# chaobrain/brainevent

Hardware: AMD Instinct MI355X
Metric: synaptic updates/sec (Geff/s), BinaryArray @ CSR scatter (higher is better)
Workload: dtype f32; 1 GPU; BinaryArray(0.01 fire) @ CSR f32 hetero, 1000000 pre x 1000000 post, 10000 synapses/row (0.01 density), route=ScatterPlan; parallelism=post-slice x1, n_post_per_gpu=1000000, n_conn=10000, stored_synapses_total=10000000000, plan_slices=51 x 19608 columns x 5 parts, layout d8 (5 B/entry)

## Files before the change

brainevent_amd/csrc/be_csr_plan.hip:

```cpp
#include "be_csr_shared.h"
#include <climits>
#include <cstring>
#ifndef BE_BLOCK_AUX
#define BE_BLOCK_AUX 2
#endif
constexpr int kD8NtMinBlock = 160;

namespace {

constexpr int kMaxSlices = 4096;

__host__ __device__ __forceinline__ uint32_t plan_group(bool homo) { return homo ? 8u : 4u; }
__host__ __device__ __forceinline__ uint32_t plan_block_units(uint32_t n_groups, bool homo) {
  const uint32_t bytes = n_groups * (homo ? 16u : 24u);
  return (bytes + 127u) >> 7;
}

__global__ void __launch_bounds__(256) k_plan_count(const int32_t* __restrict__ indices, RowPtr rp, int64_t m,
                                                    uint32_t slice_width, int n_slices, int homo, uint2* __restrict__ seg) {
  __shared__ uint32_t hist[kMaxSlices];
  for (int64_t r = blockIdx.x; r < m; r += gridDim.x) {
    for (int s = threadIdx.x; s < n_slices; s += blockDim.x) hist[s] = 0;
    __syncthreads();
    const int64_t b = rp.at(r), e = rp.at(r + 1);
// ... 133 lines not shown
#pragma unroll
    for (int off = 32; off > 0; off >>= 1) {
      const uint32_t o = __shfl_down(my_max, off, 64);
      my_max = o > my_max ? o : my_max;
    }
    if (lane_id() == 0 && my_max != 0) atomicMax(maxabs_bits, my_max);
#pragma unroll
    for (int off = 32; off > 0; off >>= 1) {
      const uint32_t o = __shfl_down(my_min, off, 64);
      my_min = o < my_min ? o : my_min;
    }
    if (lane_id() == 0 && my_min != 0xffffffffu) atomicMin(maxabs_bits + 1, my_min);
  }
}

template <int FUSED>
__device__ __forceinline__ uint32_t fused_word(const void* __restrict__ spikes, int64_t gw, int64_t m) {
  uint32_t w = 0;
  if (FUSED == 1) {
    w = static_cast<const uint32_t*>(spikes)[gw];
  } else {
    const uint8_t* sp = static_cast<const uint8_t*>(spikes) + gw * 32;
    if (gw * 32 + 32 <= m) {
      const uint4 a = reinterpret_cast<const uint4*>(sp)[0], b = reinterpret_cast<const uint4*>(sp)[1];
      const uint32_t v[8] = {a.x, a.y, a.z, a.w, b.x, b.y, b.z, b.w};
#pragma unroll
      for (int q = 0; q < 8; ++q)
#pragma unroll
        for (int e = 0; e < 4; ++e) w |= (((v[q] >> (8 * e)) & 0xffu) != 0u ? 1u : 0u) << (4 * q + e);
    } else {
      for (int e = 0; e < 32 && gw * 32 + e < m; ++e) w |= (sp[e] != 0 ? 1u : 0u) << e;
    }
  }
  const int64_t left = m - gw * 32;
  return left >= 32 ? w : (left > 0 ? (w & ((1u << (uint32_t)left) - 1u)) : 0u);
}

__device__ __forceinline__ uint32_t block_scan_total_1024(uint32_t v, uint32_t* wave_tot , uint32_t* total) {
  const int lane = threadIdx.x & 63, wave = threadIdx.x >> 6;
  uint32_t incl = v;
#pragma unroll
  for (int off = 1; off < 64; off <<= 1) {
    const uint32_t t = __shfl_up(incl, off, 64);
    if (lane >= off) incl += t;
  }
  if (lane == 63) wave_tot[wave] = incl;
  __syncthreads();
  uint32_t base = 0, t = 0;
#pragma unroll
  for (int w = 0; w < 16; ++w) {
    const uint32_t x = wave_tot[w];
    t += x;
    if (w < wave) base += x;
  }
  *total = t;
  return base + incl;
}

template <int FUSED>
__device__ __forceinline__ uint32_t build_part_list(const void* __restrict__ spikes, int64_t m, int part, int parts,
                                                    uint32_t* lds_list, uint32_t lds_cap, uint32_t* glob_list,
                                                    uint32_t* wave_tot , const uint32_t** list_out) {
  const int64_t n_words = (m + 31) >> 5;
  const int64_t n_stripes = (n_words + 31) >> 5;
  const int64_t my_words = part < n_stripes ? ((n_stripes - part + parts - 1) / parts) * 32 : 0;
  uint32_t* dst = lds_list;
  uint32_t base = 0;
  int buf = 0;
  for (int64_t u0 = 0; u0 < my_words; u0 += 1024) {
    const int64_t u = u0 + threadIdx.x;
    const int64_t gw = ((u >> 5) * parts + part) * 32 + (u & 31);
    uint32_t w = (u < my_words && gw < n_words) ? fused_word<FUSED>(spikes, gw, m) : 0u;
    const uint32_t v = __popc(w);
    uint32_t it_total;
    uint32_t pos = base + block_scan_total_1024(v, wave_tot + 16 * buf, &it_total) - v;
    buf ^= 1;
    if (dst == lds_list && base + it_total > lds_cap) {
      dst = glob_list;
      base = 0;
      u0 = -1024;
      continue;
    }
    while (w) {
      const uint32_t b = __ffs(w) - 1u;
      dst[pos++] = (uint32_t)(gw * 32) + b;
      w &= w - 1u;
    }
    base += it_total;
  }
  __syncthreads();
  *list_out = dst;
  return base;
}

__global__ void __launch_bounds__(256) k_gather_seg(const uint2* __restrict__ seg, const uint32_t* __restrict__ active,
                                                    const uint32_t* __restrict__ n_active_p, int n_slices, int64_t a_stride,
                                                    uint2* __restrict__ dense) {
  __shared__ uint2 tile[64][65];
  const uint32_t n_active = *n_active_p;
  const int lane = threadIdx.x & 63, wave = threadIdx.x >> 6;
  for (uint32_t c = blockIdx.x; (uint64_t)c * 64 < n_active; c += gridDim.x) {
    const uint32_t a0 = c * 64;
    const uint32_t n_here = n_active - a0 < 64u ? n_active - a0 : 64u;
    const uint32_t i_mine = (uint32_t)wave * 16u + (uint32_t)(lane & 15);
    const uint32_t rid = active[a0 + (i_mine < n_here ? i_mine : 0u)];
    for (int s0 = 0; s0 < n_slices; s0 += 64) {
      const int sl = s0 + lane < n_slices ? s0 + lane : n_slices - 1;
// ... 241 lines not shown
  if (L >= n_tasks) return;
  const int part = L / n_slices;
  const int slice = L - part * n_slices;
  if constexpr (FUSED == 0) active += (int64_t)blockIdx.y * active_stride;
  partial += ((int64_t)blockIdx.y * n_tasks + L) * stride;
  {
    uint4* z = reinterpret_cast<uint4*>(smem_raw);
    const int n16 = (int)(((size_t)(S + 1) * sizeof(acc_t) + 15) / 16);
    for (int i = threadIdx.x; i < n16; i += blockDim.x) z[i] = make_uint4(0u, 0u, 0u, 0u);
  }
  __syncthreads();

  __shared__ uint32_t fused_wtot[32];
  uint32_t n_active;
  if constexpr (FUSED == 1 || FUSED == 2) {
    n_active = build_part_list<FUSED>(static_cast<const unsigned char*>(fused_spikes) + (int64_t)blockIdx.y * fused_stride, fused_m,
                                      part, parts, reinterpret_cast<uint32_t*>(smem_raw + list_off), lds_cap,
                                      glob_lists + ((int64_t)blockIdx.y * parts + part) * glob_region, fused_wtot, &active);
  } else {
    n_active = n_active_p[blockIdx.y];
  }
  uint32_t pos_lo = 0;
  if constexpr (FUSED == 3) {
    const uint32_t npp = (n_active + (uint32_t)parts - 1u) / (uint32_t)parts;
    pos_lo = (uint32_t)part * npp;
    const uint32_t hi = pos_lo + npp < n_active ? pos_lo + npp : n_active;
    n_active = hi > pos_lo ? hi : pos_lo;
  }
  const uint2* sp = FUSED == 3 ? seg + (int64_t)slice * glob_region : seg + slice;
  const uint64_t seg_rs = FUSED == 3 ? 1u : (uint64_t)n_slices;
  const int wave = threadIdx.x >> 6, lane = threadIdx.x & 63, nw = blockDim.x >> 6;
  const uint64_t a0 = FUSED == 3 ? (uint64_t)pos_lo + (uint64_t)wave * 64 + lane
                      : FUSED  ? (uint64_t)wave + (uint64_t)nw * lane
// ... 400 lines not shown
  }
#pragma unroll
  for (int off = 32; off > 0; off >>= 1) {
    const uint32_t o = __shfl_down(my_max, off, 64);
    my_max = o > my_max ? o : my_max;
  }
  if (lane_id() == 0 && my_max != 0) atomicMax(maxabs_bits, my_max);
#pragma unroll
  for (int off = 32; off > 0; off >>= 1) {
    const uint32_t o = __shfl_down(my_min, off, 64);
    my_min = o < my_min ? o : my_min;
  }
  if (lane_id() == 0) atomicMin(maxabs_bits + 1, my_min);
}

__device__ __forceinline__ uint32_t wave_incl_scan_u32(uint32_t v) {
  v += (uint32_t)__builtin_amdgcn_update_dpp(0, (int)v, 0x111, 0xf, 0xf, false);
  v += (uint32_t)__builtin_amdgcn_update_dpp(0, (int)v, 0x112, 0xf, 0xf, false);
  v += (uint32_t)__builtin_amdgcn_update_dpp(0, (int)v, 0x114, 0xf, 0xf, false);
  v += (uint32_t)__builtin_amdgcn_update_dpp(0, (int)v, 0x118, 0xf, 0xf, false);
  v += (uint32_t)__builtin_amdgcn_update_dpp(0, (int)v, 0x142, 0xa, 0xf, false);
  v += (uint32_t)__builtin_amdgcn_update_dpp(0, (int)v, 0x143, 0xc, 0xf, false);
  return v;
}

__device__ __forceinline__ void d8_add4(unsigned long long* acc, uint32_t before, uint32_t d, const be_v4u& wv, float scale) {
  const uint32_t c0 = before + (d & 0xffu), c1 = c0 + ((d >> 8) & 0xffu), c2 = c1 + ((d >> 16) & 0xffu), c3 = c2 + (d >> 24);
#ifdef BE_ABL_NOATOMIC
  const unsigned long long v0 = fixed_from_f32(__uint_as_float(wv.x), scale), v1 = fixed_from_f32(__uint_as_float(wv.y), scale),
                           v2 = fixed_from_f32(__uint_as_float(wv.z), scale), v3 = fixed_from_f32(__uint_as_float(wv.w), scale);
  asm volatile("" ::"v"(c0), "v"(c1), "v"(c2), "v"(c3), "v"(v0), "v"(v1), "v"(v2), "v"(v3));
#else
  atomicAdd(&acc[c0], fixed_from_f32(__uint_as_float(wv.x), scale));
  atomicAdd(&acc[c1], fixed_from_f32(__uint_as_float(wv.y), scale));
  atomicAdd(&acc[c2], fixed_from_f32(__uint_as_float(wv.z), scale));
  atomicAdd(&acc[c3], fixed_from_f32(__uint_as_float(wv.w), scale));
#endif
}
__device__ __forceinline__ uint32_t d8_sum4(uint32_t d) { return (d & 0xffu) + ((d >> 8) & 0xffu) + ((d >> 16) & 0xffu) + (d >> 24); }

// ... 156 lines not shown
  using acc_t = unsigned long long;
  extern __shared__ __align__(16) unsigned char smem_raw[];
  acc_t* acc = reinterpret_cast<acc_t*>(smem_raw);
  const int S = cap;
#ifdef BE_PLAN_PROF
  unsigned long long plan_t = __builtin_amdgcn_s_memtime();
#endif
  const int per_xcd = gridDim.x >> 3;
  const int L = (blockIdx.x & 7) * per_xcd + (blockIdx.x >> 3);
  const int n_tasks = n_slices * parts;
  if (L >= n_tasks) return;
  const int part = L / n_slices;
  const int slice = L - part * n_slices;
  if constexpr (FUSED == 0) active += (int64_t)blockIdx.y * active_stride;
  partial += ((int64_t)blockIdx.y * n_tasks + L) * S;
  {
    uint4* z = reinterpret_cast<uint4*>(smem_raw);
    const int n16 = (int)(((size_t)(S + 1) * sizeof(acc_t) + 15) / 16);
    for (int i = threadIdx.x; i < n16; i += blockDim.x) z[i] = make_uint4(0u, 0u, 0u, 0u);
  }
  __syncthreads();
  PLAN_STAMP(0);
  __shared__ uint32_t fused_wtot[32];
  uint32_t n_active;
  if constexpr (FUSED == 1 || FUSED == 2) {
    n_active = build_part_list<FUSED>(static_cast<const unsigned char*>(fused_spikes) + (int64_t)blockIdx.y * fused_stride, fused_m,
                                      part, parts, reinterpret_cast<uint32_t*>(smem_raw + list_off), lds_cap,
                                      glob_lists + ((int64_t)blockIdx.y * parts + part) * glob_region, fused_wtot, &active);
  } else {
    n_active = n_active_p[blockIdx.y];
  }
  uint32_t pos_lo = 0;
  if constexpr (FUSED == 3) {
    const uint32_t npp = (n_active + (uint32_t)parts - 1u) / (uint32_t)parts;
    pos_lo = (uint32_t)part * npp;
    const uint32_t hi = pos_lo + npp < n_active ? pos_lo + npp : n_active;
    n_active = hi > pos_lo ? hi : pos_lo;
  }
  PLAN_STAMP(1);
  const uint2* sp = FUSED == 3 ? seg + (int64_t)slice * glob_region : seg + slice;
  const uint64_t seg_rs = FUSED == 3 ? 1u : (uint64_t)n_slices;
  const int wave = threadIdx.x >> 6, lane = threadIdx.x & 63, nw = blockDim.x >> 6;
  const uint64_t a0 = FUSED == 3 ? (uint64_t)pos_lo + (uint64_t)wave * 64 + lane
                      : FUSED  ? (uint64_t)wave + (uint64_t)nw * lane
                               : (uint64_t)part + (uint64_t)parts * ((uint64_t)wave + (uint64_t)nw * lane);
  const uint64_t a_step = FUSED ? (uint64_t)nw * 64 : (uint64_t)parts * nw * 64;
  if (n_active > pos_lo) {
    const uint64_t last = n_active - 1;
    uint64_t a = a0;
    bool v_n = a < n_active;
    uint32_t r_n = FUSED == 3 ? (uint32_t)(a < last ? a : last) : active[a < last ? a : last];
    a += a_step;
    uint2 sg = sp[(uint64_t)r_n * seg_rs];
    uint32_t st_v = sg.x, n4_v = v_n ? sg.y : 0u;
    bool v_c = v_n;
    v_n = a < n_active;
    r_n = FUSED == 3 ? (uint32_t)(a < last ? a : last) : active[a < last ? a : last];
    a += a_step;
    PLAN_STAMP(2);
    while (__ballot(v_c) != 0ull) {
      const int nvalid = __popcll(__ballot(v_c));
      const uint2 sgn = sp[(uint64_t)r_n * seg_rs];
      const bool v_nn = a < n_active;
      const uint32_t r_nn = FUSED == 3 ? (uint32_t)(a < last ? a : last) : active[a < last ? a : last];
      a += a_step;
      if constexpr (LPB > 0) {
        constexpr int BPI = 64 / LPB;
        constexpr int NGRP = 64 / BPI;
        constexpr int DEPTH = 4;
        QGroupD8 g[NGRP];
#pragma unroll
        for (int q = 0; q < DEPTH; ++q) d8q_issue<LPB>(g[q], q * BPI, nvalid, st_v, n4_v, lane, blob);
#pragma unroll
        for (int q = 0; q < NGRP; ++q) {
          if (q + DEPTH < NGRP) d8q_issue<LPB>(g[q + DEPTH], (q + DEPTH) * BPI, nvalid, st_v, n4_v, lane, blob);
          d8q_consume<LPB>(g[q], acc, lane, scale);
        }
        d8q_tails<LPB>(st_v, n4_v, nvalid, acc, lane, scale, blob);
      } else {
// ... 152 lines not shown
  const int n_tasks = n_slices * parts;
  if (L >= n_tasks) return;
  const int part = L / n_slices;
  const int slice = L - part * n_slices;
  if constexpr (FUSED == 0) active += (int64_t)blockIdx.y * active_stride;
  partial += ((int64_t)blockIdx.y * n_tasks + L) * S;
  {
    uint4* z = reinterpret_cast<uint4*>(smem_raw);
    const int n16 = (int)((size_t)S * 4 / 16);
    for (int i = threadIdx.x; i < n16; i += blockDim.x) z[i] = make_uint4(0u, 0u, 0u, 0u);
  }
  __syncthreads();
  __shared__ uint32_t fused_wtot[32];
  uint32_t n_active;
  if constexpr (FUSED == 1 || FUSED == 2) {
    n_active = build_part_list<FUSED>(static_cast<const unsigned char*>(fused_spikes) + (int64_t)blockIdx.y * fused_stride, fused_m,
                                      part, parts, reinterpret_cast<uint32_t*>(smem_raw + list_off), lds_cap,
                                      glob_lists + ((int64_t)blockIdx.y * parts + part) * glob_region, fused_wtot, &active);
  } else {
    n_active = n_active_p[blockIdx.y];
  }
  uint32_t pos_lo = 0;
  if constexpr (FUSED == 3) {
    const uint32_t npp = (n_active + (uint32_t)parts - 1u) / (uint32_t)parts;
    pos_lo = (uint32_t)part * npp;
    const uint32_t hi = pos_lo + npp < n_active ? pos_lo + npp : n_active;
    n_active = hi > pos_lo ? hi : pos_lo;
  }
  const uint2* sp = FUSED == 3 ? seg + (int64_t)slice * glob_region : seg + slice;
  const uint64_t seg_rs = FUSED == 3 ? 1u : (uint64_t)n_slices;
  const int wave = threadIdx.x >> 6, lane = threadIdx.x & 63, nw = blockDim.x >> 6;
  const uint64_t a0 = FUSED == 3 ? (uint64_t)pos_lo + (uint64_t)wave * 64 + lane
                      : FUSED  ? (uint64_t)wave + (uint64_t)nw * lane
// ... 470 lines not shown
                              (layout == BE_PLAN_H8 && slice_width <= kH8MaxWidth));
}
static inline int64_t cap_of(int slice_shift, int slice_width, int layout, int homo) {
  if (layout == BE_PLAN_D8) return (width_of(slice_shift, slice_width) + 1) & ~1ll;
  if (layout == BE_PLAN_H8) return (width_of(slice_shift, slice_width) + 3) & ~3ll;
  const int64_t w = width_of(slice_shift, slice_width);
  return homo ? (w + 3) & ~3ll : (w + 1) & ~1ll;
}
static inline int64_t lds_slots_of(int slice_shift, int slice_width, int layout, int homo) {
  return layout == BE_PLAN_U16 ? (1ll << slice_shift) : cap_of(slice_shift, slice_width, layout, homo);
}

#define COMMA ,
constexpr int kPreGatherMaxBlock = 64;
constexpr int kPreGatherMinSlices = 40;
constexpr size_t kFusedMinList = 2048;
static inline int64_t fused_region_of(int64_t m, int parts) {
  const int64_t n_stripes = (((m + 31) >> 5) + 31) >> 5;
  return ((n_stripes + parts - 1) / parts) * 1024;
}

int64_t be_scatter_plan_scratch_bytes(int64_t m, int64_t k, int slice_shift, int slice_width) {
  const int64_t n = (int64_t)n_slices_of(k, slice_shift, slice_width) * m;
  const int64_t n_blocks = (n + kScanChunk - 1) / kScanChunk;
  return be_align_up((n_blocks + 2) * 8, 256);
}

static inline unsigned long long* plan_too_long(void* scratch, int64_t m, int n_slices) {
  const int64_t n_blocks = ((int64_t)n_slices * m + kScanChunk - 1) / kScanChunk;
  return reinterpret_cast<unsigned long long*>(static_cast<uint64_t*>(scratch) + n_blocks + 1);
}
// ... 396 lines not shown
                                               int parts, int homo) {
  const int64_t n_slices = n_slices_of(k, slice_shift, slice_width);
  const int64_t acc_bytes = homo ? 4 : 8;
  const int64_t task = std::max<int64_t>(1ll << slice_shift, (width_of(slice_shift, slice_width) + 3) & ~3ll);
  return counts_bytes(n_batch) + n_batch * plan_active_stride(m) * 4 +
         be_align_up(n_batch * n_slices * parts * task * acc_bytes, 256);
}
int64_t be_binary_csrmm_t_plan_workspace_bytes_for(int64_t m, int64_t k, int64_t n_batch, int slice_shift, int slice_width,
                                                   int parts, int homo, int block_hint) {
  const int64_t base = be_binary_csrmm_t_plan_workspace_bytes(m, k, n_batch, slice_shift, slice_width, parts, homo);
  const bool pre = block_hint > 0 && block_hint <= pregather_max_block();
  return base + (pre ? plan_dense_seg_bytes(m, n_slices_of(k, slice_shift, slice_width), n_batch) : 0);
}
int64_t be_binary_csrmv_t_plan_workspace_bytes(int64_t m, int64_t k, int slice_shift, int slice_width, int parts, int homo) {
  return be_binary_csrmm_t_plan_workspace_bytes(m, k, 1, slice_shift, slice_width, parts, homo);
}

int be_binary_csrmm_t_plan(const void* weights, int homo, int wdtype, const void* blob, const void* seg,
                           const void* spikes, int spike_dtype, void* out, int64_t m, int64_t k, int64_t n_batch,
                           int slice_shift, int slice_width, int layout, int block_hint, int parts, int scale_exp,
                           void* workspace, int64_t workspace_bytes, be_stream_t stream) {
  BE_REQUIRE(m > 0 && k > 0 && m <= 0xffffffffll && k <= 0xffffffffll, BE_ERR_INVALID, "bad shape");
  BE_REQUIRE(layout == BE_PLAN_U16 || (layout == BE_PLAN_D8 && !homo) || (layout == BE_PLAN_H8 && homo), BE_ERR_INVALID,
             "bad plan layout");
  BE_REQUIRE(n_batch >= 1 && n_batch <= kMaxBatch, BE_ERR_INVALID, "n_batch out of range");
  BE_REQUIRE(slice_shift >= 4 && slice_shift <= 15, BE_ERR_INVALID, "slice_shift must be in [4, 15]");
  BE_REQUIRE(width_ok(slice_shift, slice_width, layout), BE_ERR_INVALID, "slice_width out of range for this layout");
  BE_REQUIRE(parts >= 1 && parts <= 64, BE_ERR_INVALID, "parts must be in [1, 64]");
  BE_REQUIRE(seg && spikes && out && blob, BE_ERR_INVALID, "null pointer");
  BE_REQUIRE(!homo || weights != nullptr, BE_ERR_INVALID, "missing weights");
// ... 25 lines not shown
    int rc1 = BE_ERR_INVALID;
#define BE_SINGLE(LAY, WT) rc1 = launch_plan_single<LAY, WT>(blob, seg, spikes, spike_dtype, m, k, (int)slots, sc1, isc1, weights, out, lds, st)
#define BE_SINGLE_W(LAY)                                                    \
    switch (wdtype) {                                                        \
      case BE_F32: BE_SINGLE(LAY, float); break;                             \
      case BE_F16: BE_SINGLE(LAY, __half); break;                            \
      case BE_BF16: BE_SINGLE(LAY, __hip_bfloat16); break;                   \
      default: be_set_error("planned scatter: f32 / f16 / bf16 outputs"); rc1 = BE_ERR_UNSUPPORTED; \
    }
    if (lay == 0) { BE_SINGLE_W(0) } else if (lay == 1) { BE_SINGLE_W(1) } else if (lay == 2) { BE_SINGLE_W(2) } else { BE_SINGLE_W(3) }
#undef BE_SINGLE_W
#undef BE_SINGLE
    be_prof_end(prof1, st);
    return rc1;
  }
  static const int fused_off = [] { const char* e = getenv("BE_PLAN_FUSED"); return e && e[0] == '0'; }();
  const size_t lds_room = 160 * 1024 - 1024 - lds;
  int fused = 0;
  if (!fused_off && lds + 1024 <= 160 * 1024 && lds_room >= kFusedMinList * 4) {
    if (spike_dtype == BE_SPIKE_BITS) fused = 1;
    else if (spike_dtype == BE_SPIKE_BOOL && (reinterpret_cast<uintptr_t>(spikes) & 15) == 0 && (n_batch == 1 || m % 16 == 0)) fused = 2;
  }
  const int64_t dense_bytes = plan_dense_seg_bytes(m, n_slices, n_batch);
  if (dense_bytes > 0 && block_hint > 0 && block_hint <= pregather_max_block() &&
      workspace_bytes >= be_binary_csrmm_t_plan_workspace_bytes(m, k, n_batch, slice_shift, slice_width, parts, homo) + dense_bytes)
    fused = 3;
  const uint32_t lds_cap = (fused == 1 || fused == 2) ? (uint32_t)std::min<size_t>(lds_room / 4, 32768) : 0u;
  const uint32_t list_off = (uint32_t)lds;
  const size_t lds_dyn = lds + (size_t)lds_cap * 4;
  const int64_t fused_stride = spike_dtype == BE_SPIKE_BITS ? ((m + 31) / 32) * 4 : m;
  const int64_t glob_region = fused == 3 ? astride : fused_region_of(m, parts);
  ActiveList al{active, count};
  const int pre_mode = fused != 3 ? 0 : (spike_dtype == BE_SPIKE_BITS ? 1 :
                       (spike_dtype == BE_SPIKE_BOOL && (reinterpret_cast<uintptr_t>(spikes) & 15) == 0) ? 2 : 0);
  if (fused == 0 || (fused == 3 && pre_mode == 0)) {
    int rc = be_resolve_active(spikes, spike_dtype, m, n_batch, active, astride, count, st, false, &al);
    if (rc != BE_OK) return rc;
  }
  const void* seg_used = seg;
  if (fused == 3) {
    uint2* dense = reinterpret_cast<uint2*>(static_cast<unsigned char*>(partial) +
                                            be_align_up((int64_t)n_slices * parts * S * (homo ? 4 : 8), 256));
    const unsigned cg_grid = (unsigned)(((m + 15) / 16 + 255) / 256);
    if (pre_mode == 1)
// ... 16 lines not shown
#define BE_FUSED_ARGS spikes, m, fused_stride, list_off, lds_cap, active, glob_region
#define BE_PLAN_LAUNCH(KERN, ...)                                                                              \
  do {                                                                                                         \
    auto kern__ = KERN;                                                                                        \
    BE_HIP(be_allow_lds(reinterpret_cast<const void*>(kern__), (int)lds_dyn));                                 \
    hipLaunchKernelGGL(kern__, grid, block, lds_dyn, st, static_cast<const unsigned char*>(blob),              \
                       static_cast<const uint2*>(seg_used), al.ids, al.count, __VA_ARGS__, BE_FUSED_ARGS);     \
  } while (0)
#define BE_PLAN_BY_FUSED(TMPL_A, TMPL_B, ...)                                                                 \
  do {                                                                                                         \
    if (fused == 1) BE_PLAN_LAUNCH((TMPL_A 1 TMPL_B), __VA_ARGS__);                                           \
    else if (fused == 2) BE_PLAN_LAUNCH((TMPL_A 2 TMPL_B), __VA_ARGS__);                                      \
    else if (fused == 3) BE_PLAN_LAUNCH((TMPL_A 3 TMPL_B), __VA_ARGS__);                                      \
    else BE_PLAN_LAUNCH((TMPL_A 0 TMPL_B), __VA_ARGS__);                                                      \
  } while (0)
  if (layout == BE_PLAN_H8) {
    BE_PLAN_BY_FUSED(k_plan_accumulate_h8<, >, n_slices, (int)S, parts, static_cast<uint32_t*>(partial), astride);
  } else if (homo) {
    uint32_t* pp = static_cast<uint32_t*>(partial);
    if (block_hint > 0 && block_hint <= kSub4MaxBlock) BE_PLAN_BY_FUSED(k_plan_accumulate<true COMMA 4 COMMA, >, n_slices, slice_shift, parts, scale, pp, astride, (int)S);
    else if (block_hint > 0 && block_hint <= kSub8MaxBlock) BE_PLAN_BY_FUSED(k_plan_accumulate<true COMMA 8 COMMA, >, n_slices, slice_shift, parts, scale, pp, astride, (int)S);
    else if (block_hint > 0 && block_hint <= kSub16MaxBlock) BE_PLAN_BY_FUSED(k_plan_accumulate<true COMMA 16 COMMA, >, n_slices, slice_shift, parts, scale, pp, astride, (int)S);
    else if (block_hint > 0 && block_hint <= kSub32MaxBlock) BE_PLAN_BY_FUSED(k_plan_accumulate<true COMMA 32 COMMA, >, n_slices, slice_shift, parts, scale, pp, astride, (int)S);
    else BE_PLAN_BY_FUSED(k_plan_accumulate<true COMMA 0 COMMA, >, n_slices, slice_shift, parts, scale, pp, astride, (int)S);
  } else if (layout == BE_PLAN_D8) {
    unsigned long long* pp = static_cast<unsigned long long*>(partial);
    if (block_hint > 0 && block_hint <= kD8EighthMaxBlock) BE_PLAN_BY_FUSED(k_plan_accumulate_d8<8 COMMA, >, n_slices, (int)S, parts, scale, pp, astride);
    else if (block_hint > 0 && block_hint <= kD8QuarterMaxBlock) BE_PLAN_BY_FUSED(k_plan_accumulate_d8<16 COMMA, >, n_slices, (int)S, parts, scale, pp, astride);
    else if (block_hint >= kD8NtMinBlock) BE_PLAN_BY_FUSED(k_plan_accumulate_d8<0 COMMA, COMMA BE_BLOCK_AUX>, n_slices, (int)S, parts, scale, pp, astride);
    else BE_PLAN_BY_FUSED(k_plan_accumulate_d8<0 COMMA, COMMA 0>, n_slices, (int)S, parts, scale, pp, astride);
  } else {
    unsigned long long* pw = static_cast<unsigned long long*>(partial);
    if (block_hint > 0 && block_hint <= kSubW4MaxBlock) BE_PLAN_BY_FUSED(k_plan_accumulate<false COMMA 4 COMMA, >, n_slices, slice_shift, parts, scale, pw, astride, (int)S);
    else if (block_hint > 0 && block_hint <= kSubW8MaxBlock) BE_PLAN_BY_FUSED(k_plan_accumulate<false COMMA 8 COMMA, >, n_slices, slice_shift, parts, scale, pw, astride, (int)S);
    else if (block_hint > 0 && block_hint <= kSubW16MaxBlock) BE_PLAN_BY_FUSED(k_plan_accumulate<false COMMA 16 COMMA, >, n_slices, slice_shift, parts, scale, pw, astride, (int)S);
    else if (block_hint > 0 && block_hint <= kSubW32MaxBlock) BE_PLAN_BY_FUSED(k_plan_accumulate<false COMMA 32 COMMA, >, n_slices, slice_shift, parts, scale, pw, astride, (int)S);
    else BE_PLAN_BY_FUSED(k_plan_accumulate<false COMMA 0 COMMA, >, n_slices, slice_shift, parts, scale, pw, astride, (int)S);
  }
#undef BE_PLAN_BY_FUSED
#undef BE_PLAN_LAUNCH
#undef BE_FUSED_ARGS
  be_prof_end(prof, st);
  BE_LAUNCH_CHECK();
  const int rgrid = grid_for(k, 256, n_batch >= 8 ? 256 : 2048);
  const int64_t pstride = (int64_t)n_tasks * S;
  BE_DISPATCH_W(wdtype, homo,
                hipLaunchKernelGGL((k_plan_reduce<W, HOMO>), dim3(rgrid, (unsigned)n_batch), dim3(256), 0, st,
                                   static_cast<const typename PlanAcc<HOMO>::type*>(partial), parts, n_slices, (int)S,
                                   (uint32_t)width_of(slice_shift, slice_width), k, inv_scale, static_cast<const W*>(weights), static_cast<W*>(out), pstride, count));
  BE_LAUNCH_CHECK();
  return BE_OK;
}

// ... 10 lines not shown
```

include/brainevent_amd.h:

```cpp
#ifndef BRAINEVENT_AMD_H
#define BRAINEVENT_AMD_H

#include <stdint.h>

#ifdef __cplusplus
extern "C" {
#endif

#define BE_OK 0
#define BE_ERR_INVALID (-1)
#define BE_ERR_WORKSPACE (-2)
#define BE_ERR_HIP (-3)
#define BE_ERR_RANGE (-4)
#define BE_ERR_UNSUPPORTED (-5)

#define BE_F32 0
#define BE_F64 1
#define BE_F16 2
#define BE_BF16 3
#define BE_SPIKE_BOOL 0
#define BE_SPIKE_FLOAT 1
#define BE_SPIKE_BITS 2
#define BE_SPIKE_IDS 3
typedef struct be_spike_ids {
// ... 126 lines not shown
int64_t be_fixed_point_scratch_bytes(int64_t k);
int be_weight_stats(const void* weights, int wdtype, int64_t n, uint32_t* max_bits_host, uint32_t* min_nonzero_bits_host,
                    void* scratch, int64_t scratch_bytes, be_stream_t stream);
int be_fixed_point_exponent(const void* weights, int wdtype, const int32_t* indices, int64_t nnz, int64_t k,
                            int min_weight_bits, int keep_exp, void* scratch, int64_t scratch_bytes, int* scale_exp_host,
                            be_stream_t stream);
int be_scatter_plan_exponent(const void* blob, const void* seg, int64_t m, int64_t k, int slice_shift, int slice_width, int layout,
                             int64_t nnz, const uint32_t* maxabs_bits, int min_weight_bits, int keep_exp, void* scratch,
                             int64_t scratch_bytes, int* scale_exp_host, be_stream_t stream);

int64_t be_binary_csrmv_t_plan_workspace_bytes(int64_t m, int64_t k, int slice_shift, int slice_width, int parts, int homo);
int64_t be_binary_csrmm_t_plan_workspace_bytes(int64_t m, int64_t k, int64_t n_batch, int slice_shift, int slice_width,
                                               int parts, int homo);
int64_t be_binary_csrmm_t_plan_workspace_bytes_for(int64_t m, int64_t k, int64_t n_batch, int slice_shift, int slice_width,
                                                   int parts, int homo, int block_hint);
int be_binary_csrmv_t_plan(const void* weights, int homo, int wdtype, const void* blob, const void* seg,
                           const void* spikes, int spike_dtype, void* out, int64_t m, int64_t k, int slice_shift,
                           int slice_width, int layout, int block_hint, int parts, int scale_exp, void* workspace,
                           int64_t workspace_bytes, be_stream_t stream);
int be_binary_csrmm_t_plan(const void* weights, int homo, int wdtype, const void* blob, const void* seg,
                           const void* spikes_bm, int spike_dtype, void* out_bm, int64_t m, int64_t k, int64_t n_batch,
                           int slice_shift, int slice_width, int layout, int block_hint, int parts, int scale_exp,
                           void* workspace, int64_t workspace_bytes, be_stream_t stream);

int be_binned_bins(int64_t k, int slice_shift, int homo);
int be_binned_set_tuning(int task_groups, int min_tasks);
int be_binned_workspace_status(const void* workspace, int clear, be_stream_t stream);
int be_binned_workspace_audit(const void* workspace, uint64_t* counters_host, be_stream_t stream);
int64_t be_binary_csrmv_t_binned_workspace_bytes(int64_t m, int64_t k, int slice_shift, int64_t bin_capacity);
int be_binary_csrmv_t_binned_workspace_init(void* workspace, int64_t workspace_bytes, int64_t m, int64_t k, int slice_shift,
// ... 187 lines not shown
```

Baseline: 816.3 Geff/s.

## Build compact 16-bit active lists and overlap accumulator zeroing in fused d8 plan

Adds fused modes 4/5 for the wave-level d8 accumulate kernel. In these modes each part's active-row list is kept in LDS as 16-bit offsets plus a few bound markers, which halves LDS use and lets longer lists stay on-chip. The list build now loads several spike words per thread, converts byte spikes to bits with dot4, uses DPP-based wave scans with two 16-bit counts packed per lane, and zeroes the accumulator while the spike loads are in flight. The cost is an extra decode step for every row lookup and more register pressure, and mode selection is moved into a new exported helper.

```diff
diff --git a/brainevent_amd/csrc/be_csr_plan.hip b/brainevent_amd/csrc/be_csr_plan.hip
--- a/brainevent_amd/csrc/be_csr_plan.hip
+++ b/brainevent_amd/csrc/be_csr_plan.hip
@@ -171,83 +171,154 @@
   }
 }
 
-template <int FUSED>
-__device__ __forceinline__ uint32_t fused_word(const void* __restrict__ spikes, int64_t gw, int64_t m) {
+__device__ __forceinline__ uint32_t wave_incl_scan_u32(uint32_t v) {
+  v += (uint32_t)__builtin_amdgcn_update_dpp(0, (int)v, 0x111, 0xf, 0xf, false);
+  v += (uint32_t)__builtin_amdgcn_update_dpp(0, (int)v, 0x112, 0xf, 0xf, false);
+  v += (uint32_t)__builtin_amdgcn_update_dpp(0, (int)v, 0x114, 0xf, 0xf, false);
+  v += (uint32_t)__builtin_amdgcn_update_dpp(0, (int)v, 0x118, 0xf, 0xf, false);
+  v += (uint32_t)__builtin_amdgcn_update_dpp(0, (int)v, 0x142, 0xa, 0xf, false);
+  v += (uint32_t)__builtin_amdgcn_update_dpp(0, (int)v, 0x143, 0xc, 0xf, false);
+  return v;
+}
+
+__device__ __forceinline__ uint32_t block_scan_waves_1024(uint32_t wave_total, int wave , uint32_t* wave_tot ,
+                                                          uint32_t* total) {
+  const int lane = threadIdx.x & 63;
+  if (lane == 0) wave_tot[wave] = wave_total;
+  __syncthreads();
+  const uint32_t x = wave_tot[lane & 15];
+  const uint32_t incl = wave_incl_scan_u32(lane < 16 ? x : 0u);
+  *total = (uint32_t)__builtin_amdgcn_readlane((int)incl, 15);
+  return wave ? (uint32_t)__builtin_amdgcn_readlane((int)incl, wave - 1) : 0u;
+}
+
+template <int SRC> struct ListWords { static constexpr int n = SRC == 1 ? 8 : 7; };
+constexpr int kListBounds = 8;
+
+template <int SRC> struct SpikeRaw { uint32_t w; };
+template <> struct SpikeRaw<2> { uint4 a, b; };
+
+template <int SRC>
+__device__ __forceinline__ void spike_raw_load(SpikeRaw<SRC>& r, const void* __restrict__ spikes, int64_t gw, int64_t m) {
+  if constexpr (SRC == 1) {
+    r.w = static_cast<const uint32_t*>(spikes)[gw];
+  } else {
+    const int64_t last = (m - 1) >> 4, c = gw * 2;
+    const uint4* p = static_cast<const uint4*>(spikes);
+    r.a = p[c];
+    r.b = p[c + 1 < last ? c + 1 : last];
+  }
+}
+
+__device__ __forceinline__ uint32_t nonzero_bytes(uint32_t v) { return (((v & 0x7f7f7f7fu) + 0x7f7f7f7fu) | v) & 0x80808080u; }
+
+template <int SRC>
+__device__ __forceinline__ uint32_t spike_raw_bits(const SpikeRaw<SRC>& r, int64_t gw, int64_t m) {
   uint32_t w = 0;
-  if (FUSED == 1) {
-    w = static_cast<const uint32_t*>(spikes)[gw];
+  if constexpr (SRC == 1) {
+    w = r.w;
   } else {
-    const uint8_t* sp = static_cast<const uint8_t*>(spikes) + gw * 32;
-    if (gw * 32 + 32 <= m) {
-      const uint4 a = reinterpret_cast<const uint4*>(sp)[0], b = reinterpret_cast<const uint4*>(sp)[1];
-      const uint32_t v[8] = {a.x, a.y, a.z, a.w, b.x, b.y, b.z, b.w};
-#pragma unroll
-      for (int q = 0; q < 8; ++q)
-#pragma unroll
-        for (int e = 0; e < 4; ++e) w |= (((v[q] >> (8 * e)) & 0xffu) != 0u ? 1u : 0u) << (4 * q + e);
-    } else {
-      for (int e = 0; e < 32 && gw * 32 + e < m; ++e) w |= (sp[e] != 0 ? 1u : 0u) << e;
+    const uint32_t v[8] = {r.a.x, r.a.y, r.a.z, r.a.w, r.b.x, r.b.y, r.b.z, r.b.w};
+#pragma unroll
+    for (int j = 0; j < 4; ++j) {
+      uint32_t x = __builtin_amdgcn_udot4(nonzero_bytes(v[2 * j]), 0x08040201u, 0u, false);
+      x = __builtin_amdgcn_udot4(nonzero_bytes(v[2 * j + 1]), 0x80402010u, x, false);
+      w |= (x >> 7) << (8 * j);
     }
   }
   const int64_t left = m - gw * 32;
   return left >= 32 ? w : (left > 0 ? (w & ((1u << (uint32_t)left) - 1u)) : 0u);
 }
 
-__device__ __forceinline__ uint32_t block_scan_total_1024(uint32_t v, uint32_t* wave_tot , uint32_t* total) {
-  const int lane = threadIdx.x & 63, wave = threadIdx.x >> 6;
-  uint32_t incl = v;
-#pragma unroll
-  for (int off = 1; off < 64; off <<= 1) {
-    const uint32_t t = __shfl_up(incl, off, 64);
-    if (lane >= off) incl += t;
-  }
-  if (lane == 63) wave_tot[wave] = incl;
-  __syncthreads();
-  uint32_t base = 0, t = 0;
-#pragma unroll
-  for (int w = 0; w < 16; ++w) {
-    const uint32_t x = wave_tot[w];
-    t += x;
-    if (w < wave) base += x;
-  }
-  *total = t;
-  return base + incl;
-}
-
-template <int FUSED>
+template <int SRC, bool C16, typename Between>
 __device__ __forceinline__ uint32_t build_part_list(const void* __restrict__ spikes, int64_t m, int part, int parts,
                                                     uint32_t* lds_list, uint32_t lds_cap, uint32_t* glob_list,
-                                                    uint32_t* wave_tot , const uint32_t** list_out) {
+                                                    uint32_t* wave_tot , uint32_t* bounds ,
+                                                    const uint32_t** list_out, bool* compact, Between between) {
+  constexpr int KW = ListWords<SRC>::n, KP = (KW + 1) / 2;
   const int64_t n_words = (m + 31) >> 5;
   const int64_t n_stripes = (n_words + 31) >> 5;
   const int64_t my_words = part < n_stripes ? ((n_stripes - part + parts - 1) / parts) * 32 : 0;
-  uint32_t* dst = lds_list;
+  if (C16 && threadIdx.x < kListBounds) bounds[threadIdx.x] = 0xffffffffu;
+  uint16_t* const lds16 = reinterpret_cast<uint16_t*>(lds_list);
+  const int lane = threadIdx.x & 63, wave = __builtin_amdgcn_readfirstlane((int)(threadIdx.x >> 6));
+  bool to_lds = true, between_done = false;
   uint32_t base = 0;
   int buf = 0;
-  for (int64_t u0 = 0; u0 < my_words; u0 += 1024) {
-    const int64_t u = u0 + threadIdx.x;
-    const int64_t gw = ((u >> 5) * parts + part) * 32 + (u & 31);
-    uint32_t w = (u < my_words && gw < n_words) ? fused_word<FUSED>(spikes, gw, m) : 0u;
-    const uint32_t v = __popc(w);
-    uint32_t it_total;
-    uint32_t pos = base + block_scan_total_1024(v, wave_tot + 16 * buf, &it_total) - v;
+  int64_t u0 = 0;
+  while (u0 < my_words) {
+    const int64_t rest = my_words - u0;
+    const int W = rest >= (int64_t)1024 * KW ? KW : (int)((rest + 1023) >> 10);
+    const int64_t ub = u0 + (int64_t)wave * W * 64 + lane;
+    SpikeRaw<SRC> raw[KW];
+    int64_t gws[KW];
+#pragma unroll
+    for (int j = 0; j < KW; ++j) {
+      const int64_t u = (j < W && ub + 64 * j < my_words) ? ub + 64 * j : u0;
+      const int64_t gw = ((u >> 5) * parts + part) * 32 + (u & 31);
+      gws[j] = gw < n_words ? gw : n_words - 1;
+      spike_raw_load<SRC>(raw[j], spikes, gws[j], m);
+    }
+    if (!between_done) {
+      between();
+      between_done = true;
+    }
+    uint32_t w[KW];
+#pragma unroll
+    for (int j = 0; j < KW; ++j) {
+      const int64_t u = ub + 64 * j;
+      const bool mine = j < W && u < my_words && ((u >> 5) * parts + part) * 32 + (u & 31) < n_words;
+      w[j] = mine ? spike_raw_bits<SRC>(raw[j], gws[j], m) : 0u;
+    }
+    uint32_t incl[KP], wave_total = 0;
+#pragma unroll
+    for (int i = 0; i < KP; ++i) {
+      incl[i] = wave_incl_scan_u32((uint32_t)__popc(w[2 * i]) | (2 * i + 1 < KW ? (uint32_t)__popc(w[2 * i + 1]) << 16 : 0u));
+      const uint32_t t = (uint32_t)__builtin_amdgcn_readlane((int)incl[i], 63);
+      wave_total += (t & 0xffffu) + (t >> 16);
+    }
+    uint32_t total;
+    uint32_t run = base + block_scan_waves_1024(wave_total, wave, wave_tot + 16 * buf, &total);
     buf ^= 1;
-    if (dst == lds_list && base + it_total > lds_cap) {
-      dst = glob_list;
+    if (to_lds && base + total > lds_cap) {
+      to_lds = false;
       base = 0;
-      u0 = -1024;
+      u0 = 0;
       continue;
     }
-    while (w) {
-      const uint32_t b = __ffs(w) - 1u;
-      dst[pos++] = (uint32_t)(gw * 32) + b;
-      w &= w - 1u;
-    }
-    base += it_total;
-  }
+#pragma unroll
+    for (int j = 0; j < KW; ++j) {
+      const int64_t u = ub + 64 * j;
+      const uint32_t sh = 16u * (uint32_t)(j & 1);
+      uint32_t pos = run + ((incl[j >> 1] >> sh) & 0xffffu) - (uint32_t)__popc(w[j]);
+      run += ((uint32_t)__builtin_amdgcn_readlane((int)incl[j >> 1], 63) >> sh) & 0xffffu;
+      if (C16 && to_lds && j < W && u < my_words && u > 0 && (u & 2047) == 0 && (u >> 11) <= kListBounds)
+        bounds[(u >> 11) - 1] = pos;
+      uint32_t x = w[j];
+      while (x) {
+        const uint32_t b = __ffs(x) - 1u;
+        if (C16 && to_lds) lds16[pos++] = (uint16_t)((uint32_t)(u * 32) + b);
+        else (to_lds ? lds_list : glob_list)[pos++] = (uint32_t)(gws[j] * 32) + b;
+        x &= x - 1u;
+      }
+    }
+    base += total;
+    u0 += (int64_t)1024 * KW;
+  }
+  if (!between_done) between();
   __syncthreads();
-  *list_out = dst;
+  *list_out = to_lds ? lds_list : glob_list;
+  *compact = C16 && to_lds;
   return base;
+}
+
+__device__ __forceinline__ uint32_t part_list_row(const uint32_t* list, const uint16_t* lds16, uint64_t i, bool compact,
+                                                  const uint32_t* bounds, uint32_t part, uint32_t parts) {
+  if (!compact) return list[i];
+  uint32_t q = lds16[i];
+#pragma unroll
+  for (int b = 0; b < kListBounds; ++b) q += (uint32_t)i >= bounds[b] ? 65536u : 0u;
+  return (((q >> 10) * parts + part) << 10) | (q & 1023u);
 }
 
 __global__ void __launch_bounds__(256) k_gather_seg(const uint2* __restrict__ seg, const uint32_t* __restrict__ active,
@@ -519,9 +590,11 @@
   __shared__ uint32_t fused_wtot[32];
   uint32_t n_active;
   if constexpr (FUSED == 1 || FUSED == 2) {
-    n_active = build_part_list<FUSED>(static_cast<const unsigned char*>(fused_spikes) + (int64_t)blockIdx.y * fused_stride, fused_m,
-                                      part, parts, reinterpret_cast<uint32_t*>(smem_raw + list_off), lds_cap,
-                                      glob_lists + ((int64_t)blockIdx.y * parts + part) * glob_region, fused_wtot, &active);
+    bool compact;
+    n_active = build_part_list<FUSED, false>(static_cast<const unsigned char*>(fused_spikes) + (int64_t)blockIdx.y * fused_stride, fused_m,
+                                             part, parts, reinterpret_cast<uint32_t*>(smem_raw + list_off), lds_cap,
+                                             glob_lists + ((int64_t)blockIdx.y * parts + part) * glob_region, fused_wtot, nullptr,
+                                             &active, &compact, [] {});
   } else {
     n_active = n_active_p[blockIdx.y];
   }
@@ -952,16 +1025,6 @@
   if (lane_id() == 0) atomicMin(maxabs_bits + 1, my_min);
 }
 
-__device__ __forceinline__ uint32_t wave_incl_scan_u32(uint32_t v) {
-  v += (uint32_t)__builtin_amdgcn_update_dpp(0, (int)v, 0x111, 0xf, 0xf, false);
-  v += (uint32_t)__builtin_amdgcn_update_dpp(0, (int)v, 0x112, 0xf, 0xf, false);
-  v += (uint32_t)__builtin_amdgcn_update_dpp(0, (int)v, 0x114, 0xf, 0xf, false);
-  v += (uint32_t)__builtin_amdgcn_update_dpp(0, (int)v, 0x118, 0xf, 0xf, false);
-  v += (uint32_t)__builtin_amdgcn_update_dpp(0, (int)v, 0x142, 0xa, 0xf, false);
-  v += (uint32_t)__builtin_amdgcn_update_dpp(0, (int)v, 0x143, 0xc, 0xf, false);
-  return v;
-}
-
 __device__ __forceinline__ void d8_add4(unsigned long long* acc, uint32_t before, uint32_t d, const be_v4u& wv, float scale) {
   const uint32_t c0 = before + (d & 0xffu), c1 = c0 + ((d >> 8) & 0xffu), c2 = c1 + ((d >> 16) & 0xffu), c3 = c2 + (d >> 24);
 #ifdef BE_ABL_NOATOMIC
@@ -1148,22 +1211,42 @@
   const int slice = L - part * n_slices;
   if constexpr (FUSED == 0) active += (int64_t)blockIdx.y * active_stride;
   partial += ((int64_t)blockIdx.y * n_tasks + L) * S;
-  {
+  auto zero_acc = [&] {
     uint4* z = reinterpret_cast<uint4*>(smem_raw);
     const int n16 = (int)(((size_t)(S + 1) * sizeof(acc_t) + 15) / 16);
     for (int i = threadIdx.x; i < n16; i += blockDim.x) z[i] = make_uint4(0u, 0u, 0u, 0u);
-  }
-  __syncthreads();
-  PLAN_STAMP(0);
+  };
   __shared__ uint32_t fused_wtot[32];
+  __shared__ uint32_t fused_bounds[kListBounds];
+  constexpr bool LISTS = FUSED == 1 || FUSED == 2 || FUSED == 4 || FUSED == 5;
+  uint32_t* const lds_list = reinterpret_cast<uint32_t*>(smem_raw + list_off);
+  bool compact = false;
   uint32_t n_active;
-  if constexpr (FUSED == 1 || FUSED == 2) {
-    n_active = build_part_list<FUSED>(static_cast<const unsigned char*>(fused_spikes) + (int64_t)blockIdx.y * fused_stride, fused_m,
-                                      part, parts, reinterpret_cast<uint32_t*>(smem_raw + list_off), lds_cap,
-                                      glob_lists + ((int64_t)blockIdx.y * parts + part) * glob_region, fused_wtot, &active);
+  if constexpr (FUSED == 4 || FUSED == 5) {
+    n_active = build_part_list<FUSED - 3, true>(static_cast<const unsigned char*>(fused_spikes) + (int64_t)blockIdx.y * fused_stride,
+                                                fused_m, part, parts, lds_list, lds_cap,
+                                                glob_lists + ((int64_t)blockIdx.y * parts + part) * glob_region, fused_wtot,
+                                                fused_bounds, &active, &compact, zero_acc);
+    PLAN_STAMP(0);
   } else {
-    n_active = n_active_p[blockIdx.y];
-  }
+    zero_acc();
+    __syncthreads();
+    PLAN_STAMP(0);
+    if constexpr (FUSED == 1 || FUSED == 2) {
+      n_active = build_part_list<FUSED, false>(static_cast<const unsigned char*>(fused_spikes) + (int64_t)blockIdx.y * fused_stride, fused_m,
+                                               part, parts, lds_list, lds_cap,
+                                               glob_lists + ((int64_t)blockIdx.y * parts + part) * glob_region, fused_wtot, nullptr,
+                                               &active, &compact, [] {});
+    } else {
+      n_active = n_active_p[blockIdx.y];
+    }
+  }
+  auto row_at = [&](uint64_t i) -> uint32_t {
+    if constexpr (FUSED == 3) return (uint32_t)i;
+    else if constexpr (FUSED == 4 || FUSED == 5)
+      return part_list_row(active, reinterpret_cast<const uint16_t*>(lds_list), i, compact, fused_bounds, (uint32_t)part, (uint32_t)parts);
+    else return active[i];
+  };
   uint32_t pos_lo = 0;
   if constexpr (FUSED == 3) {
     const uint32_t npp = (n_active + (uint32_t)parts - 1u) / (uint32_t)parts;
@@ -1176,27 +1259,27 @@
   const uint64_t seg_rs = FUSED == 3 ? 1u : (uint64_t)n_slices;
   const int wave = threadIdx.x >> 6, lane = threadIdx.x & 63, nw = blockDim.x >> 6;
   const uint64_t a0 = FUSED == 3 ? (uint64_t)pos_lo + (uint64_t)wave * 64 + lane
-                      : FUSED  ? (uint64_t)wave + (uint64_t)nw * lane
+                      : LISTS  ? (uint64_t)wave + (uint64_t)nw * lane
                                : (uint64_t)part + (uint64_t)parts * ((uint64_t)wave + (uint64_t)nw * lane);
   const uint64_t a_step = FUSED ? (uint64_t)nw * 64 : (uint64_t)parts * nw * 64;
   if (n_active > pos_lo) {
     const uint64_t last = n_active - 1;
     uint64_t a = a0;
     bool v_n = a < n_active;
-    uint32_t r_n = FUSED == 3 ? (uint32_t)(a < last ? a : last) : active[a < last ? a : last];
+    uint32_t r_n = row_at(a < last ? a : last);
     a += a_step;
     uint2 sg = sp[(uint64_t)r_n * seg_rs];
     uint32_t st_v = sg.x, n4_v = v_n ? sg.y : 0u;
     bool v_c = v_n;
     v_n = a < n_active;
-    r_n = FUSED == 3 ? (uint32_t)(a < last ? a : last) : active[a < last ? a : last];
+    r_n = row_at(a < last ? a : last);
     a += a_step;
     PLAN_STAMP(2);
     while (__ballot(v_c) != 0ull) {
       const int nvalid = __popcll(__ballot(v_c));
       const uint2 sgn = sp[(uint64_t)r_n * seg_rs];
       const bool v_nn = a < n_active;
-      const uint32_t r_nn = FUSED == 3 ? (uint32_t)(a < last ? a : last) : active[a < last ? a : last];
+      const uint32_t r_nn = row_at(a < last ? a : last);
       a += a_step;
       if constexpr (LPB > 0) {
         constexpr int BPI = 64 / LPB;
@@ -1379,9 +1462,11 @@
   __shared__ uint32_t fused_wtot[32];
   uint32_t n_active;
   if constexpr (FUSED == 1 || FUSED == 2) {
-    n_active = build_part_list<FUSED>(static_cast<const unsigned char*>(fused_spikes) + (int64_t)blockIdx.y * fused_stride, fused_m,
-                                      part, parts, reinterpret_cast<uint32_t*>(smem_raw + list_off), lds_cap,
-                                      glob_lists + ((int64_t)blockIdx.y * parts + part) * glob_region, fused_wtot, &active);
+    bool compact;
+    n_active = build_part_list<FUSED, false>(static_cast<const unsigned char*>(fused_spikes) + (int64_t)blockIdx.y * fused_stride, fused_m,
+                                             part, parts, reinterpret_cast<uint32_t*>(smem_raw + list_off), lds_cap,
+                                             glob_lists + ((int64_t)blockIdx.y * parts + part) * glob_region, fused_wtot, nullptr,
+                                             &active, &compact, [] {});
   } else {
     n_active = n_active_p[blockIdx.y];
   }
@@ -1882,7 +1967,8 @@
 #define COMMA ,
 constexpr int kPreGatherMaxBlock = 64;
 constexpr int kPreGatherMinSlices = 40;
-constexpr size_t kFusedMinList = 2048;
+constexpr size_t kFusedMinIds = 2048;
+constexpr size_t kList32MinRoom = kFusedMinIds * 4, kList16MinRoom = kFusedMinIds * 2;
 static inline int64_t fused_region_of(int64_t m, int parts) {
   const int64_t n_stripes = (((m + 31) >> 5) + 31) >> 5;
   return ((n_stripes + parts - 1) / parts) * 1024;
@@ -2309,6 +2395,39 @@
 }
 int64_t be_binary_csrmv_t_plan_workspace_bytes(int64_t m, int64_t k, int slice_shift, int slice_width, int parts, int homo) {
   return be_binary_csrmm_t_plan_workspace_bytes(m, k, 1, slice_shift, slice_width, parts, homo);
+}
+
+int be_scatter_plan_step_mode(int64_t m, int64_t k, int64_t n_batch, int slice_shift, int slice_width, int layout, int block_hint,
+                              int parts, int homo, int spike_dtype, int spike_addr_low4, int64_t workspace_bytes) {
+  BE_REQUIRE(m > 0 && k > 0 && m <= 0xffffffffll && k <= 0xffffffffll, BE_ERR_INVALID, "bad shape");
+  BE_REQUIRE(layout == BE_PLAN_U16 || (layout == BE_PLAN_D8 && !homo) || (layout == BE_PLAN_H8 && homo), BE_ERR_INVALID,
+             "bad plan layout");
+  BE_REQUIRE(n_batch >= 1 && n_batch <= kMaxBatch, BE_ERR_INVALID, "n_batch out of range");
+  BE_REQUIRE(slice_shift >= 4 && slice_shift <= 15, BE_ERR_INVALID, "slice_shift must be in [4, 15]");
+  BE_REQUIRE(width_ok(slice_shift, slice_width, layout), BE_ERR_INVALID, "slice_width out of range for this layout");
+  BE_REQUIRE(parts >= 1 && parts <= 64, BE_ERR_INVALID, "parts must be in [1, 64]");
+  const int64_t slots = lds_slots_of(slice_shift, slice_width, layout, homo);
+  const size_t lds = ((size_t)(slots + 1) * (homo ? 4 : 8) + 15) & ~(size_t)15;
+  BE_REQUIRE(lds <= 160 * 1024, BE_ERR_RANGE, "slice does not fit LDS (hetero: slice_shift <= 14)");
+  static const int fused_off = [] { const char* e = getenv("BE_PLAN_FUSED"); return e && e[0] == '0'; }();
+  const int n_slices = n_slices_of(k, slice_shift, slice_width);
+  int fused = 0;
+  if (!fused_off && lds + 1024 <= 160 * 1024) {
+    const size_t lds_room = 160 * 1024 - 1024 - lds;
+    const bool bits = spike_dtype == BE_SPIKE_BITS;
+    const bool bytes = spike_dtype == BE_SPIKE_BOOL && (spike_addr_low4 & 15) == 0 && (n_batch == 1 || m % 16 == 0);
+    const bool wave_d8 = layout == BE_PLAN_D8 && !(block_hint > 0 && block_hint <= kD8QuarterMaxBlock);
+    const bool list16 = n_batch == 1 && wave_d8 && fused_region_of(m, parts) <= (int64_t)(kListBounds + 1) << 16;
+    if (bits || bytes) {
+      if (list16 && lds_room >= kList16MinRoom) fused = bits ? 4 : 5;
+      else if (lds_room >= kList32MinRoom) fused = bits ? 1 : 2;
+    }
+  }
+  const int64_t dense_bytes = plan_dense_seg_bytes(m, n_slices, n_batch);
+  if (dense_bytes > 0 && block_hint > 0 && block_hint <= pregather_max_block() &&
+      workspace_bytes >= be_binary_csrmm_t_plan_workspace_bytes(m, k, n_batch, slice_shift, slice_width, parts, homo) + dense_bytes)
+    fused = 3;
+  return fused;
 }
 
 int be_binary_csrmm_t_plan(const void* weights, int homo, int wdtype, const void* blob, const void* seg,
@@ -2364,20 +2483,15 @@
     be_prof_end(prof1, st);
     return rc1;
   }
-  static const int fused_off = [] { const char* e = getenv("BE_PLAN_FUSED"); return e && e[0] == '0'; }();
   const size_t lds_room = 160 * 1024 - 1024 - lds;
-  int fused = 0;
-  if (!fused_off && lds + 1024 <= 160 * 1024 && lds_room >= kFusedMinList * 4) {
-    if (spike_dtype == BE_SPIKE_BITS) fused = 1;
-    else if (spike_dtype == BE_SPIKE_BOOL && (reinterpret_cast<uintptr_t>(spikes) & 15) == 0 && (n_batch == 1 || m % 16 == 0)) fused = 2;
-  }
-  const int64_t dense_bytes = plan_dense_seg_bytes(m, n_slices, n_batch);
-  if (dense_bytes > 0 && block_hint > 0 && block_hint <= pregather_max_block() &&
-      workspace_bytes >= be_binary_csrmm_t_plan_workspace_bytes(m, k, n_batch, slice_shift, slice_width, parts, homo) + dense_bytes)
-    fused = 3;
-  const uint32_t lds_cap = (fused == 1 || fused == 2) ? (uint32_t)std::min<size_t>(lds_room / 4, 32768) : 0u;
+  const int fused = be_scatter_plan_step_mode(m, k, n_batch, slice_shift, slice_width, layout, block_hint, parts, homo, spike_dtype,
+                                              (int)(reinterpret_cast<uintptr_t>(spikes) & 15), workspace_bytes);
+  if (fused < 0) return fused;
+  const bool list16 = fused == 4 || fused == 5;
+  const uint32_t lds_cap = (fused == 1 || fused == 2) ? (uint32_t)std::min<size_t>(lds_room / 4, 32768)
+                           : list16                   ? (uint32_t)std::min<size_t>(lds_room / 2, 65536) : 0u;
   const uint32_t list_off = (uint32_t)lds;
-  const size_t lds_dyn = lds + (size_t)lds_cap * 4;
+  const size_t lds_dyn = lds + (size_t)lds_cap * (list16 ? 2 : 4);
   const int64_t fused_stride = spike_dtype == BE_SPIKE_BITS ? ((m + 31) / 32) * 4 : m;
   const int64_t glob_region = fused == 3 ? astride : fused_region_of(m, parts);
   ActiveList al{active, count};
@@ -2424,6 +2538,15 @@
     else if (fused == 3) BE_PLAN_LAUNCH((TMPL_A 3 TMPL_B), __VA_ARGS__);                                      \
     else BE_PLAN_LAUNCH((TMPL_A 0 TMPL_B), __VA_ARGS__);                                                      \
   } while (0)
+#define BE_PLAN_BY_FUSED_D8W(TMPL_A, TMPL_B, ...)                                                             \
+  do {                                                                                                         \
+    if (fused == 4) BE_PLAN_LAUNCH((TMPL_A 4 TMPL_B), __VA_ARGS__);                                           \
+    else if (fused == 5) BE_PLAN_LAUNCH((TMPL_A 5 TMPL_B), __VA_ARGS__);                                      \
+    else if (fused == 1) BE_PLAN_LAUNCH((TMPL_A 1 TMPL_B), __VA_ARGS__);                                      \
+    else if (fused == 2) BE_PLAN_LAUNCH((TMPL_A 2 TMPL_B), __VA_ARGS__);                                      \
+    else if (fused == 3) BE_PLAN_LAUNCH((TMPL_A 3 TMPL_B), __VA_ARGS__);                                      \
+    else BE_PLAN_LAUNCH((TMPL_A 0 TMPL_B), __VA_ARGS__);                                                      \
+  } while (0)
   if (layout == BE_PLAN_H8) {
     BE_PLAN_BY_FUSED(k_plan_accumulate_h8<, >, n_slices, (int)S, parts, static_cast<uint32_t*>(partial), astride);
   } else if (homo) {
@@ -2437,8 +2560,8 @@
     unsigned long long* pp = static_cast<unsigned long long*>(partial);
     if (block_hint > 0 && block_hint <= kD8EighthMaxBlock) BE_PLAN_BY_FUSED(k_plan_accumulate_d8<8 COMMA, >, n_slices, (int)S, parts, scale, pp, astride);
     else if (block_hint > 0 && block_hint <= kD8QuarterMaxBlock) BE_PLAN_BY_FUSED(k_plan_accumulate_d8<16 COMMA, >, n_slices, (int)S, parts, scale, pp, astride);
-    else if (block_hint >= kD8NtMinBlock) BE_PLAN_BY_FUSED(k_plan_accumulate_d8<0 COMMA, COMMA BE_BLOCK_AUX>, n_slices, (int)S, parts, scale, pp, astride);
-    else BE_PLAN_BY_FUSED(k_plan_accumulate_d8<0 COMMA, COMMA 0>, n_slices, (int)S, parts, scale, pp, astride);
+    else if (block_hint >= kD8NtMinBlock) BE_PLAN_BY_FUSED_D8W(k_plan_accumulate_d8<0 COMMA, COMMA BE_BLOCK_AUX>, n_slices, (int)S, parts, scale, pp, astride);
+    else BE_PLAN_BY_FUSED_D8W(k_plan_accumulate_d8<0 COMMA, COMMA 0>, n_slices, (int)S, parts, scale, pp, astride);
   } else {
     unsigned long long* pw = static_cast<unsigned long long*>(partial);
     if (block_hint > 0 && block_hint <= kSubW4MaxBlock) BE_PLAN_BY_FUSED(k_plan_accumulate<false COMMA 4 COMMA, >, n_slices, slice_shift, parts, scale, pw, astride, (int)S);
@@ -2447,6 +2570,7 @@
     else if (block_hint > 0 && block_hint <= kSubW32MaxBlock) BE_PLAN_BY_FUSED(k_plan_accumulate<false COMMA 32 COMMA, >, n_slices, slice_shift, parts, scale, pw, astride, (int)S);
     else BE_PLAN_BY_FUSED(k_plan_accumulate<false COMMA 0 COMMA, >, n_slices, slice_shift, parts, scale, pw, astride, (int)S);
   }
+#undef BE_PLAN_BY_FUSED_D8W
 #undef BE_PLAN_BY_FUSED
 #undef BE_PLAN_LAUNCH
 #undef BE_FUSED_ARGS
diff --git a/include/brainevent_amd.h b/include/brainevent_amd.h
--- a/include/brainevent_amd.h
+++ b/include/brainevent_amd.h
@@ -164,6 +164,9 @@
                                                int parts, int homo);
 int64_t be_binary_csrmm_t_plan_workspace_bytes_for(int64_t m, int64_t k, int64_t n_batch, int slice_shift, int slice_width,
                                                    int parts, int homo, int block_hint);
+int be_scatter_plan_step_mode(int64_t m, int64_t k, int64_t n_batch, int slice_shift, int slice_width, int layout,
+                              int block_hint, int parts, int homo, int spike_dtype, int spike_addr_low4,
+                              int64_t workspace_bytes);
 int be_binary_csrmv_t_plan(const void* weights, int homo, int wdtype, const void* blob, const void* seg,
                            const void* spikes, int spike_dtype, void* out, int64_t m, int64_t k, int slice_shift,
                            int slice_width, int layout, int block_hint, int parts, int scale_exp, void* workspace,
```

Result: slower. 802.6 Geff/s (-1.7%).
